# JuliaQuantumControl/QuOptimalControl.jl

Measured on AMD Instinct MI355X. Metric: GRAPE gradient-evals/sec, higher is better.
Workload: dtype f64; 1 GPU; C3: UnitaryGate 4x4, K=4, N=500 slices, ensemble E=1024 (one GPU, 1024 members/GPU), T=2.0; step = host->host grape_eval; parallelism=single GPU

## Files before the change

### quoptimalcontrol.jl_amd/csrc/grape_api.cpp

```cpp
#include "../../include/grape_hip.h"

#include <hip/hip_runtime.h>
#include <rccl/rccl.h>

#include <dlfcn.h>
#include <fcntl.h>
#include <time.h>
#include <unistd.h>

#include <algorithm>
#include <cmath>
#include <complex>
#include <cstdio>
#include <cstdlib>
#include <cstring>
#include <limits>
#include <atomic>
#include <condition_variable>
#include <mutex>
#include <thread>
#include <new>
#include <utility>
#include <string>
#include <vector>
// ... 21 lines not shown
    int any_blocks = 1;
    size_t scratch_bytes = 0;
    bool grid = false;
    int EU = 0;
    int S = 0, W = 0, LT = 0;
    bool pair = false;
    int CH = 0;
    int MPB = 1, NB = 0;
    int B = 1;
    double *d_block_out = nullptr;
    double *d_xg_scratch = nullptr;
    int ksplit = 1;
    size_t ws_elems = 0;
    int Ec = 0, EUc = 0;
    size_t ws_unit = 0;
    size_t ws_budget = 0;
    int ws_arrays = 1;
    bool ws_invalid = false;
    bool ws_keep_costates = false;
    int test_fail_replan = 0;
    int ws_B = 1;
    uint64_t bytes = 0;
    double2 *d_ops = nullptr;
    double *d_wts = nullptr;
    double *d_x = nullptr;
    double *d_fg = nullptr;
    double2 *d_props = nullptr, *d_states = nullptr, *d_costates = nullptr;
    double *d_zphi = nullptr;
    bool exact_w1 = false;
    double *d_member_out = nullptr;
    double *d_partial = nullptr;
    double *d_fom_member = nullptr, *d_fom_rows = nullptr;
    unsigned long long *d_stamps = nullptr;
    double *h_stage = nullptr;
    double *d_h_stage = nullptr;
    double *h_fg = nullptr;
    double *d_h_fg = nullptr;
    unsigned long long *h_flag = nullptr, *d_h_flag = nullptr;
    int mf_wait = 0;
    unsigned *d_done_counter = nullptr;
    bool peer_sum = false;
    bool peer_direct = false;
    bool peer_all = false;
    double *d_gather = nullptr;
    hipEvent_t ev_done = nullptr;
    unsigned *d_arrive = nullptr;
// ... 399 lines not shown
        if (w->th.joinable()) w->th.join();
        delete w;
        c->worker = nullptr;
    }
    for (grape_ctx *s : c->sub) free_all(s);
    c->sub.clear();
    if (c->is_group) {
        if (c->d_gather) { (void)hipSetDevice(c->device); (void)hipFree(c->d_gather); }
        if (c->d_arrive) { (void)hipSetDevice(c->device); (void)hipFree(c->d_arrive); }
        if (c->d_basis_phi) { (void)hipSetDevice(c->device); (void)hipFree(c->d_basis_phi); (void)hipFree(c->d_basis_x0); }
        if (c->d_bounds || c->d_slope) { (void)hipSetDevice(c->device); (void)hipFree(c->d_bounds); (void)hipFree(c->d_slope); }
        delete c;
        return;
    }
    (void)hipSetDevice(c->device);
    for (int j = 0; j < c->ipc_ranks; ++j)
        if (c->ipc_mbox[j] && c->ipc_mbox[j] != c->d_mbox) (void)hipIpcCloseMemHandle(c->ipc_mbox[j]);
    if (c->d_mbox) (void)hipFree(c->d_mbox);
    if (c->comm && g_rccl.handle) (void)g_rccl.CommDestroy(c->comm);
    for (hipEvent_t e : c->ev) (void)hipEventDestroy(e);
    if (c->ev_dev) (void)hipEventDestroy(c->ev_dev);
    if (c->ev_done) (void)hipEventDestroy(c->ev_done);
    if (c->stream) (void)hipStreamDestroy(c->stream);
    (void)hipFree(c->d_ops); (void)hipFree(c->d_wts); (void)hipFree(c->d_x); (void)hipFree(c->d_fg);
    (void)hipFree(c->d_props); (void)hipFree(c->d_states); (void)hipFree(c->d_costates); (void)hipFree(c->d_zphi);
    (void)hipFree(c->d_ctrl_scale);
    (void)hipFree(c->d_member_out); (void)hipFree(c->d_partial); (void)hipFree(c->d_stamps); (void)hipFree(c->d_block_out); (void)hipFree(c->d_xg_scratch);
    if (c->h_stage) (void)hipHostFree(c->h_stage);
    if (c->h_fg) (void)hipHostFree(c->h_fg);
    if (c->h_flag) (void)hipHostFree(c->h_flag);
    (void)hipFree(c->d_done_counter);
    (void)hipFree(c->d_scratch);
    (void)hipFree(c->d_vecs);
    (void)hipFree(c->d_sp_coef); (void)hipFree(c->d_sp_addr);
    (void)hipFree(c->d_any_sp_i); (void)hipFree(c->d_any_sp_c);
    (void)hipFree(c->d_tp_q); (void)hipFree(c->d_tp_r); (void)hipFree(c->d_tp_m); (void)hipFree(c->d_tp_z); (void)hipFree(c->d_tp_vec); (void)hipFree(c->d_tp_a);
    (void)hipFree(c->d_x_bar);
    (void)hipFree(c->d_pen_w);
    (void)hipFree(c->d_rc_R); (void)hipFree(c->d_rc_rho); (void)hipFree(c->d_rc_xs); (void)hipFree(c->d_rc_rows);
    (void)hipFree(c->d_obs_O); (void)hipFree(c->d_obs_y); (void)hipFree(c->d_obs_xf);
    (void)hipFree(c->d_vjp_O); (void)hipFree(c->d_vjp_ybar); (void)hipFree(c->d_vjp_xbar); (void)hipFree(c->d_vjp_part); (void)hipFree(c->d_vjp_g); (void)hipFree(c->d_vjp_out);
    (void)hipFree(c->d_traj_w); (void)hipFree(c->d_traj_x);
    (void)hipFree(c->d_jvp_O); (void)hipFree(c->d_jvp_xdot); (void)hipFree(c->d_jvp_xphys); (void)hipFree(c->d_jvp_ydot); (void)hipFree(c->d_jvp_xf);
    (void)hipFree(c->d_basis_phi); (void)hipFree(c->d_basis_x0);
    (void)hipFree(c->d_bounds); (void)hipFree(c->d_slope);
    (void)hipFree(c->d_fom_member); (void)hipFree(c->d_fom_rows);
    (void)hipFree(c->d_risk_rows); (void)hipFree(c->d_risk_p);
// ... 247 lines not shown
    if (e == hipSuccess && c->family == 0) e = alloc((void **)&c->d_block_out, sizeof(double) * c->NB * Q * Bn);
    if (e == hipSuccess && c->family == 0 && !xg_in_lds)
        e = alloc((void **)&c->d_xg_scratch,
                  sizeof(double) * Bn * c->NB * ((size_t)c->MPB * c->CH * ((size_t)S * K + 1) + c->MPB));
    if (e == hipSuccess && (cfg->flags & GRAPE_FLAG_PHASE_STAMPS)) {
        const size_t sb = sizeof(unsigned long long) * Bn * E * W * grape::kStampSlots;
        e = alloc((void **)&c->d_stamps, sb);
        if (e == hipSuccess) e = hipMemset(c->d_stamps, 0, sb);
    }
    const unsigned hflags = hipHostMallocMapped | hipHostMallocCoherent | hipHostMallocPortable;
    if (e == hipSuccess) e = hipHostMalloc((void **)&c->h_stage, sizeof(double) * Q * Bn, hflags);
    if (e == hipSuccess) e = hipHostGetDevicePointer((void **)&c->d_h_stage, c->h_stage, 0);
    if (e == hipSuccess) e = hipHostMalloc((void **)&c->h_fg, sizeof(double) * Q * Bn, hflags);
    if (e == hipSuccess) e = hipHostGetDevicePointer((void **)&c->d_h_fg, c->h_fg, 0);
    if (e == hipSuccess) e = hipHostMalloc((void **)&c->h_flag, 64 + sizeof(unsigned long long) * grape::kMaxMflags, hflags);
    if (e == hipSuccess) e = hipHostGetDevicePointer((void **)&c->d_h_flag, c->h_flag, 0);
    if (e == hipSuccess) { std::memset(c->h_flag, 0, 64 + sizeof(unsigned long long) * grape::kMaxMflags); e = alloc((void **)&c->d_done_counter, 64); }
    if (e == hipSuccess) e = hipMemset(c->d_done_counter, 0, 64);
    {
        const char *dp = std::getenv("GRAPE_DIRECT_PUBLISH");
        c->direct_publish = !(dp && dp[0] == '0');
        c->mf_publish = !env_off("GRAPE_MF_PUBLISH");
        c->pair_ah_env = !env_off("GRAPE_PAIR_AH");
    }
    {
        const char *xu = std::getenv("GRAPE_X_UPLOAD");
        int mode = 2;
        if (xu) mode = !std::strcmp(xu, "memcpy") ? 0 : (!std::strcmp(xu, "kernel") ? 1 : 2);
        int large_bar = 0;
        if (mode == 2 && e == hipSuccess &&
            (hipDeviceGetAttribute(&large_bar, hipDeviceAttributeIsLargeBar, dev) != hipSuccess || !large_bar))
            mode = 1;
        if (mode == 2 && e == hipSuccess) {
            void *p = nullptr;
            if (hipExtMallocWithFlags(&p, sizeof(double) * KN(c) * Bn, hipDeviceMallocFinegrained) == hipSuccess && p) {
                const int fd = open("/dev/zero", O_RDONLY);
                const bool ok = fd >= 0 && read(fd, p, 64) == 64;
                if (fd >= 0) close(fd);
                if (ok) {
                    c->d_x_bar = (double *)p;
                    c->bytes += sizeof(double) * KN(c) * Bn;
                } else {
                    (void)hipFree(p);
                    mode = 1;
                }
            } else {
// ... 1186 lines not shown
        if (c->tp_C) {
            const size_t bytes = sizeof(double2) * nn * (size_t)c->cfg.n_ensemble * c->B * (size_t)c->tp_C;
            const char *what = "the time chunks' products";
            if (int rc = grow(c, &c->d_tp_q, &c->tp_cap[0], bytes, who, what)) return rc;
            if (int rc = grow(c, &c->d_tp_r, &c->tp_cap[1], bytes, who, what)) return rc;
            if (int rc = grow(c, &c->d_tp_m, &c->tp_cap[2], bytes, who, what)) return rc;
        }
        const size_t need = per_block * (size_t)std::max(c->any_blocks, std::max(1, c->tp_C));
        if (int rc = grow(c, &c->d_scratch, &c->scratch_bytes, need, who, "the propagator blocks' scratch matrices")) return rc;
    }
    if (thin) {
        c->unitary = false;
        if (!c->d_vecs) {
            c->bytes += sizeof(double) * E * 4 * VS;
            HIP_TRY(c, hipMalloc((void **)&c->d_vecs, sizeof(double) * E * 4 * VS));
        }
        HIP_TRY(c, hipMemcpy(c->d_vecs, vecs.data(), sizeof(double) * E * 4 * VS, hipMemcpyHostToDevice));
        const size_t rec = sizeof(double2) * (size_t)c->Ec * ((size_t)c->cfg.n_slices + 1) * VS * ws_batch(c);
        if (int rc = grow(c, &c->d_states, &c->states_bytes, rec, who, "the forward states")) return rc;
    } else if (!herm || c->exact_w1) {
        if (int rc = grow(c, &c->d_states, &c->states_bytes, sizeof(double2) * c->ws_elems * ws_batch(c), who, "the forward states")) return rc;
    }
    HIP_TRY(c, hipMemcpy(c->d_ops, packed.data(), sizeof(double) * packed.size(), hipMemcpyHostToDevice));
    HIP_TRY(c, hipMemcpy(c->d_wts, wts, sizeof(double) * E, hipMemcpyHostToDevice));
    c->h_wts.assign(wts, wts + E);
    c->ops_set = true;
    c->evaluated = false;
    c->risk_evaluated = false;
    return GRAPE_OK;
}

static TileParams tile_params(const grape_ctx *c, const double *d_x, int n_x = 1)
{
    TileParams p{};
    p.n_x = n_x;
    p.ops = c->d_ops;
    p.x = d_x;
    p.props = c->d_props;
    p.states = c->d_states;
    p.costates = c->d_costates;
    p.member_out = c->d_member_out;
    p.K = c->cfg.n_controls;
    p.N = c->cfg.n_slices;
    p.E = c->EU;
    p.E_plan = c->EU;
    p.E_members = c->cfg.n_ensemble;
// ... 74 lines not shown
    if (pen_active(c)) {
        d.pen_x = d_x;
        d.pen_w = c->d_pen_w;
        d.pen_K = c->cfg.n_controls;
        d.pen_N = c->cfg.n_slices;
    }
    return d;
}

static grape::DoneSignal host_signal(grape_ctx *s, double *host_out)
{
    grape::DoneSignal d;
    d.counter = s->d_done_counter;
    d.flag = s->d_h_flag;
    d.seq = ++s->seq;
    d.host_out = host_out;
    return d;
}

static SweepParams sweep_params(const grape_ctx *c, const double *d_x, int n_x)
{
    SweepParams p{};
    p.ops = c->d_ops;
    p.x = d_x;
    p.wts = c->d_wts;
    p.MPB = c->MPB;
    p.BPX = c->NB;
    p.n_x = n_x;
    p.sk_magic = (uint32_t)((1ull << 32) / ((uint64_t)c->S * c->cfg.n_controls)) + 1u;
    p.K = c->cfg.n_controls;
    p.N = c->cfg.n_slices;
    p.E = c->cfg.n_ensemble;
    p.S = c->S;
    p.LT = c->LT;
    p.s_forced = c->cfg.expm_squarings;
    p.variant = c->cfg.variant;
    p.dt = c->cfg.duration / c->cfg.n_slices;
    return p;
}

static bool pair_antiherm(const grape_ctx *c)
{
    return c->family == 0 && c->pair && c->unitary && c->cfg.n == 4 && c->cfg.sys_type == GRAPE_UNITARY_GATE && !c->exact_w1 &&
           c->cfg.gradient != GRAPE_GRADIENT_EXACT && c->pair_ah_env;
}

// ... 269 lines not shown
        const size_t slot = (size_t)(c->ev_issued % kEventRing);
        e0 = c->ev[3 * slot];
        e1 = c->ev[3 * slot + 2];
        if (c->family == 1 || (c->family == 2 && c->any_blocks > 1)) emid = c->ev[3 * slot + 1];
        c->ev_has_mid[slot] = emid ? 1 : 0;
        c->ev_issued += 1;
        HIP_TRY(c, hipEventRecord(e0, stream));
    }
    const bool exact = c->cfg.gradient == GRAPE_GRADIENT_EXACT;
    if (exact) p.member_out = nullptr;
    const bool direct = c->family == 0 && c->NB == 1 && n_x == 1 && !exact && c->direct_publish && !done.probe_out &&
                        !done.stage_base && !pen_active(c) && !rc_on && !risk;
    const bool fold = !done.stage_base && tile_folds_reduce(c, n_x);
    if (direct) {
        p.direct_dst = done.flag && done.host_out ? done.host_out : d_fg;
        p.direct_flag = done.flag;
        p.direct_seq = done.seq;
    }
    const size_t nn = (size_t)c->cfg.n * c->cfg.n, Kc = (size_t)c->cfg.n_controls, Qrow = KN(c) + 1;
    auto launch_members = [&](int lo, int cnt) -> int {
        if (c->family == 0) {
            SweepParams q = p;
            q.ops = p.ops + (size_t)lo * (Kc + 3) * nn;
            q.wts = p.wts + lo;
            if (p.member_out) q.member_out = p.member_out + (size_t)lo * Qrow;
            q.block_out = p.block_out + (size_t)(lo / c->MPB) * Qrow;
            if (p.zphi) q.zphi = p.zphi + 2 * (size_t)lo;
            q.E = cnt;
            q.BPX = (cnt + c->MPB - 1) / c->MPB;
            const int mode = c->unitary ? 2 : (c->d_costates ? 1 : 0), sand = c->cfg.sys_type != GRAPE_UNITARY_GATE;
            HIP_TRY(c, launch_small_family(c, sand, (mode == 2 && pair_antiherm(c)) ? 3 : mode, q, stream));
            if (rc_on) {
                SweepParams r = q;
                r.rc_only = 1;
                r.rc_terms = c->rc_terms;
                r.rc_m = c->m;
                r.rc_unitary = c->unitary ? 1 : 0;
                r.rc_CH = c->CH;
                r.rc_Etot = c->cfg.n_ensemble;
                r.rc_R = c->d_rc_R + (size_t)lo * c->cfg.n * c->m;
                r.rc_rho = c->d_rc_rho;
                r.rc_xs = c->d_rc_xs;
                r.rc_rows = c->d_rc_rows;
                if (c->rc_mode == GRAPE_TRAJ_EXACT) {
                    r.rc_exact = 1;
                    r.traj_w = c->d_traj_w;
// ... 2126 lines not shown
```

### quoptimalcontrol.jl_amd/csrc/grape_kernels.hpp

```cpp
#pragma once
#include <hip/hip_runtime.h>
#include <stddef.h>
#include <stdint.h>
#include <type_traits>

namespace grape {

void log_kernel(const char *expr);
#define GRAPE_LAUNCH(KERNEL, ...)                        \
    do {                                                 \
        ::grape::log_kernel(#KERNEL);                    \
        hipLaunchKernelGGL(KERNEL, __VA_ARGS__);         \
    } while (0)
#define GRAPE_LAUNCH_AS(NAME, KERNEL, ...)               \
    do {                                                 \
        ::grape::log_kernel(NAME);                       \
        hipLaunchKernelGGL(KERNEL, __VA_ARGS__);         \
    } while (0)


constexpr double kTheta8 = 0.08;

struct BasisOp {
    int32_t project = 0;
// ... 8 lines not shown
};
struct DoneSignal {
    unsigned *counter = nullptr;
    unsigned long long *flag = nullptr;
    unsigned long long seq = 0;
    double *host_out = nullptr;
    const double *stage_base = nullptr;
    int n_total = 0;
    const double *probe_dir = nullptr;
    const double *probe_sc = nullptr;
    double *probe_out = nullptr;
    unsigned long long *mflags = nullptr;
    const double *pen_x = nullptr;
    const double *pen_w = nullptr;
    int pen_K = 0, pen_N = 0;
    const BasisOp *basis = nullptr;
    double risk_beta = 0.0;
    double *risk_p = nullptr;
    double *risk_F = nullptr;
};
constexpr int kMaxMflags = 1000;
int reduce_rows_mflags(int Q, int n_x);

constexpr int kStampSlots = 8;

struct SweepParams {
    const double2 *ops;
    const double *x;
    double2 *props;
    double2 *states;
    double2 *costates;
    double *member_out;
    const double *wts;
    double *block_out;
    unsigned long long *stamps;
    double *xg_scratch;
    int32_t K, N, E;
    int32_t S;
    int32_t LT;
    int32_t MPB;
    int32_t BPX;
    int32_t n_x;
    uint32_t sk_magic;
    int32_t s_forced;
    int32_t variant;
    int32_t plast_lds;
    double dt;
// ... 44 lines not shown
    double *vjp_part;
    double *vjp_G;
    int32_t obs_staged;
    int32_t vjp_staged;
    int32_t jvp_only;
    int32_t jvp_n;
    int32_t jvp_m;
    int32_t jvp_per_member;
    int32_t jvp_CH;
    int32_t jvp_Etot;
    int32_t jvp_E0;
    const double2 *jvp_O;
    const double *jvp_xdot;
    double2 *jvp_ydot;
    double2 *jvp_xf;
    int32_t traj_exact;
    double2 *traj_w;
    const double *traj_x;
    int32_t rc_exact;
    int32_t rc_unweighted;
    int32_t jvp_ndir;
    int32_t jvp_multi;
    int64_t jvp_dir_xdot, jvp_dir_ydot, jvp_dir_xf, jvp_dir_w;
};
constexpr int kJvpMultiMaxThreads = 256;
constexpr int jvp_multi_block(int n, int m)
{
    return n == 2 ? 8 : n == 3 ? 4 : n == 4 ? (m <= 2 ? 3 : 2) : 0;
}
constexpr bool jvp_multi_default(int n, int m)
{
    return jvp_multi_block(n, m) > 0;
}
constexpr int traj_max_threads(int n)
{
    return n == 2 ? 1024 : n == 3 ? 512 : 256;
}
constexpr size_t traj_static_lds(int n, int m, bool vjp)
{
    return (size_t)(traj_max_threads(n) / 64) * (size_t)(n * n + (vjp ? n * m : 0)) * 16;
}
template <typename F>
hipError_t dispatch_nm(int n, int m, F &&f)
{
#define GRAPE_NM_CASE(N, M) \
    case N * 8 + M: return f(std::integral_constant<int, N>{}, std::integral_constant<int, M>{})
    switch (n * 8 + m) {
// ... 225 lines not shown
```

### quoptimalcontrol.jl_amd/csrc/sweep_pair.hip

```cpp
#include "cmatp.hpp"
#include "grape_kernels.hpp"

#ifndef GRAPE_ABL
#define GRAPE_ABL 0
#endif
#ifndef GRAPE_PD
#define GRAPE_PD 2
#endif
#ifndef GRAPE_PLAYOUT
#define GRAPE_PLAYOUT 0
#endif
#ifndef GRAPE_PD_EARLY
#define GRAPE_PD_EARLY 2
#endif
#ifndef GRAPE_PD_EARLY_AT
#define GRAPE_PD_EARLY_AT 0
#endif
#ifndef GRAPE_MBAR
#define GRAPE_MBAR 2
#endif

namespace grape {

enum { PMODE_GENERAL = 0, PMODE_GENERAL_KEEPL = 1, PMODE_UNITARY = 2, PMODE_UNITARY_AH = 3 };
constexpr int kAhImage = 5;
constexpr int kParityPad = 8;

template <int N>
GRAPE_DEV int gelem(int q, int r, int jl)
{
    constexpr int NC = N / 2;
    const int i = (((r / NC) ^ q) * NC) + (r % NC);
    const int j = q * NC + jl;
    return i + j * N;
}

template <int N>
GRAPE_DEV void pstore_ws(double2 *__restrict__ base, size_t stride, const PMat<N> &m, int q)
{
#pragma unroll
    for (int jl = 0; jl < N / 2; ++jl)
#pragma unroll
        for (int r = 0; r < N; ++r)
            base[(size_t)gelem<N>(q, r, jl) * stride] = make_double2(m.re[r + jl * N], m.im[r + jl * N]);
}

template <int N>
GRAPE_DEV void pstore_ws_split(double2 *__restrict__ sbase, const unsigned (&voff)[2], size_t stride, const PMat<N> &m)
{
// ... 191 lines not shown
    for (int c = 0; c < K; c += 2) {
        if (c + 1 < K) {
#pragma unroll
            for (int e = 0; e < kAhImage; ++e)
                b1[e] = s_img[(c + 1) * kAhImage + e];
        }
        const double re = dot(b0);
        if (p == 0)
            out[c] = gs * re;
        if (c + 1 < K) {
            if (c + 2 < K) {
#pragma unroll
                for (int e = 0; e < kAhImage; ++e)
                    b0[e] = s_img[(c + 2) * kAhImage + e];
            }
            const double r1 = dot(b1);
            if (p == 0)
                out[c + 1] = gs * r1;
        }
    }
}

constexpr int kVecSlices = 16;
template <int N, int SAND, int MODE, int MAXT, bool XGLDS, bool DUMPW = false, bool VEC = false>
__global__ __launch_bounds__(MAXT) void sweep_pair_kernel(const double2 *__restrict__ ops_all,
                                                          const double *__restrict__ x_all,
                                                          const double *__restrict__ wts_all,
                                                          const SweepParams p)
{
    constexpr int NN = N * N, NC = N / 2, NE = N * NC;
    constexpr int MAXW = MAXT / 64;
    constexpr bool AH = (MODE == PMODE_UNITARY_AH);
    constexpr bool UNI = (MODE == PMODE_UNITARY) || AH;
    constexpr bool KEEPL = (MODE == PMODE_GENERAL_KEEPL);
    static_assert(!AH || (N == 4 && !SAND && !DUMPW && !VEC), "the anti-Hermitian sweep serves UnitaryGate at n = 4, first-order gradient");
    constexpr bool PDASM = (GRAPE_PD == 2) && UNI && N == 4 && !DUMPW && XGLDS;
    extern __shared__ double2 s_dyn[];
    double2(*s_tot)[MAXW][NN] = reinterpret_cast<double2(*)[MAXW][NN]>(s_dyn);

    const int LT = p.LT, W = LT >> 6, CH = LT >> 1;
    const int mb = __builtin_amdgcn_readfirstlane(threadIdx.x / LT);
    const int L = threadIdx.x - mb * LT;
    const int lane = L & 63, wave = L >> 6;
    const int par = L & 1;
    const int ch = L >> 1;
    const int cw = lane >> 1;
    const int wbase_tot = mb * W;
    const int xi = blockIdx.x / p.BPX;
    const int bi = blockIdx.x - xi * p.BPX;
    int kl = bi * p.MPB + mb;
    const bool valid = kl < p.E;
    if (!valid)
        kl = p.E - 1;
    const int k = xi * p.E + kl;
    const int K = p.K, Nsl = p.N, S = p.S;
    const size_t stride = (size_t)CH;
    const int NM = 2 * K + 4;

    unsigned *s_cnt = reinterpret_cast<unsigned *>(s_dyn + 2 * MAXW * NN);
    double2 *s_ops_all = s_dyn + 2 * MAXW * NN + 4;
    const int PS = NM * NE + kParityPad;
    double2 *s_ops = s_ops_all + (size_t)mb * 2 * PS;
    const int SK = S * K;
    const size_t nrm_d2 = ((size_t)p.MPB * (K + 1) + 1) / 2;
    double *s_xg_all = XGLDS ? reinterpret_cast<double *>(s_ops_all + (size_t)p.MPB * 2 * PS + nrm_d2)
                             : p.xg_scratch + (size_t)blockIdx.x * ((size_t)p.MPB * CH * (SK + 1) + p.MPB);
    double *s_xg = s_xg_all + (size_t)mb * CH * (SK + 1);
    double *s_F = s_xg_all + (size_t)p.MPB * CH * (SK + 1);
    double2 *s_plast = reinterpret_cast<double2 *>(s_F + ((p.MPB + 1) & ~1));
    double *s_nrm = reinterpret_cast<double *>(s_ops_all + (size_t)p.MPB * 2 * PS) + (size_t)mb * (K + 1);
    const unsigned magic = p.sk_magic;
    auto chunk_of = [&](int q) { return SK == 1 ? q : (int)__umulhi((unsigned)q, magic); };
    if (threadIdx.x < 16)
        s_cnt[threadIdx.x] = 0u;
    if (p.tune & 7) {
        const int sel = p.tune & 7;
        const bool hi = sel == 1 ? (mb & 1) : sel == 2 ? (mb & 2) : sel == 3 ? (blockIdx.x & 1) : sel == 4 ? ((threadIdx.x >> 6) & 1) : false;
        if (hi)
            __builtin_amdgcn_s_setprio(2);
    }
    {
        const double *__restrict__ xsrc = x_all + (size_t)xi * K * Nsl;
        const int KNs = K * Nsl;
        for (int q0 = 0; q0 < KNs; q0 += 8 * LT) {
            double v[8];
#pragma unroll
            for (int u = 0; u < 8; ++u) {
                const int q = q0 + u * LT + L;
                v[u] = q < KNs ? xsrc[q] : 0.0;
            }
#pragma unroll
            for (int u = 0; u < 8; ++u) {
                const int q = q0 + u * LT + L;
                if (q < KNs)
                    s_xg[q + chunk_of(q)] = v[u];
            }
        }
        const double2 *__restrict__ ops = ops_all + (size_t)kl * (K + 3) * NN;
        for (int idx = L; idx < 2 * NM * NE; idx += LT) {
            const int q = idx / (NM * NE), rem = idx - q * NM * NE;
            const int mat = rem / NE, e = rem - mat * NE;
            if (mat == 2 * K + 3 || (AH && mat > K && mat <= 2 * K))
                continue;
// ... 34 lines not shown
        double sr = 0.0, si = 0.0;
        for (int kk = 0; kk < N; ++kk) {
            const double2 a = gXi[i + kk * N], b = gXt[j + kk * N];
            sr = fma(a.x, b.x, sr); sr = fma(a.y, b.y, sr);
            si = fma(a.y, b.x, si); si = fma(-a.x, b.y, si);
        }
        s_ops[(size_t)q * PS + (size_t)(2 * K + 3) * NE + e] = make_double2(sr, si);
    }
    __syncthreads();
    if (L <= K) {
        double best = 0.0;
        for (int q = 0; q < 2; ++q)
            for (int jl = 0; jl < NC; ++jl) {
                double cs = 0.0;
                for (int r = 0; r < N; ++r) {
                    const double2 v = s_ops[(size_t)q * PS + (size_t)L * NE + r + jl * N];
                    cs += fabs(v.x) + fabs(v.y);
                }
                best = fmax(best, cs);
            }
        s_nrm[L] = best;
    }
    __syncthreads();
    const double2 *sA = s_ops + (size_t)par * PS;
    const double2 *sB = sA + NE;
    const double2 *sBT = sA + (size_t)(1 + K) * NE;
    const double2 *sXi = sA + (size_t)(1 + 2 * K) * NE;
    const double2 *sXt = sXi + NE;
    const double2 *sXi_o = s_ops + (size_t)(1 - par) * PS + (size_t)(1 + 2 * K) * NE;
    const double2 *sXt_o = sXi_o + NE;
    const double2 *sXX = sXt + NE, *sXX_o = sXt_o + NE;
    double *xg = s_xg + ch * (SK + 1);
    const size_t wbase = (size_t)k * S * NN * stride + ch;
    const size_t pstep = GRAPE_PLAYOUT ? (size_t)p.E * p.n_x * NN * stride : (size_t)NN * stride;
    double2 *__restrict__ Pw = p.props + (GRAPE_PLAYOUT ? (size_t)k * NN * stride + ch : wbase);
    double2 *__restrict__ Xw = p.states + wbase;
    double *__restrict__ out = p.member_out + (size_t)k * ((size_t)K * Nsl + 1);
    const int t0 = ch * S;
    const unsigned p_rowb = (unsigned)CH * 16u;
    const unsigned p_voff[2] = {(unsigned)(par * NC + par * NC * N) * p_rowb + (unsigned)ch * 16u,
                                (unsigned)((1 - par) * NC + par * NC * N) * p_rowb + (unsigned)ch * 16u};
    double2 *__restrict__ const p_Pk = p.props + (size_t)k * (GRAPE_PLAYOUT ? 1 : S) * NN * stride;
    unsigned long long *__restrict__ st =
        p.stamps ? p.stamps + ((size_t)k * W + wave) * kStampSlots : nullptr;
    if (st && lane == 0)
        st[5] = __builtin_amdgcn_s_memrealtime();
    pstamp(st, 0);

    PMat<N> Q, Q2;
    auto build = [&](int j, PMat<N> &G) -> double {
        double nb = s_nrm[0];
        double2 b0[NE], b1[NE];
#pragma unroll
        for (int e = 0; e < NE; ++e)
            b0[e] = sB[e];
        if (p.variant != 0)
            pload_lds(G, sA);
        for (int c = 0; c < K; c += 2) {
            const int c1 = min(c + 1, K - 1), c2 = min(c + 2, K - 1);
            const double x0 = xg[j * K + c];
            const double x1 = (c + 1 < K) ? xg[j * K + c1] : 0.0;
            nb = fma(fabs(x0), s_nrm[1 + c], nb);
            nb = fma(fabs(x1), s_nrm[1 + c1], nb);
#pragma unroll
            for (int e = 0; e < NE; ++e)
                b1[e] = sB[c1 * NE + e];
            if (c == 0 && p.variant == 0) {
#pragma unroll
                for (int e = 0; e < NE; ++e) {
// ... 681 lines not shown
            for (int m = 0; m < nmem; ++m) {
                const double v = (q < KN) ? s_xg_all[m * mstride + off] : s_F[m];
                acc = fma(v, wb[m], acc);
            }
            bout[q] = acc;
            if (p.direct_dst)
                p.direct_dst[q] = acc;
        }
    }
    if (p.direct_flag) {
        __threadfence_system();
        __syncthreads();
        if (threadIdx.x == 0)
            __hip_atomic_store(p.direct_flag, p.direct_seq, __ATOMIC_RELEASE, __HIP_MEMORY_SCOPE_SYSTEM);
    }
    pstamp(st, 4);
    if (st && lane == 0) {
        st[6] = __builtin_amdgcn_s_memrealtime();
        st[7] = ((unsigned long long)__builtin_amdgcn_s_getreg(20 | (31 << 11)) << 32) |
                (unsigned)__builtin_amdgcn_s_getreg(4 | (31 << 11));
    }
}

template <int N>
struct PairTraits;
template <> struct PairTraits<2> { static constexpr int MAXT = 1024; };
template <> struct PairTraits<4> { static constexpr int MAXT = 512; };

int sweep_pair_max_waves(int n)
{
    switch (n) {
    case 2: return PairTraits<2>::MAXT / 64;
    case 4: return PairTraits<4>::MAXT / 64;
    default: return 0;
    }
}

size_t sweep_pair_lds_bytes(int n, int MPB, int LT, int S, int K, bool xg_in_lds, bool plast)
{
    const int maxt = n == 2 ? PairTraits<2>::MAXT : PairTraits<4>::MAXT;
    size_t b = sizeof(double2) * (2 * (size_t)(maxt / 64) * n * n + 4);
    b += sizeof(double2) * ((size_t)MPB * 2 * ((2 * K + 4) * (n * (n / 2)) + kParityPad) + ((size_t)MPB * (K + 1) + 1) / 2);
    if (xg_in_lds)
        b += sizeof(double) * ((size_t)MPB * (LT / 2) * ((size_t)S * K + 1) + ((MPB + 1) & ~1));
    if (plast)
        b += sizeof(double2) * (size_t)MPB * LT * (n * (n / 2));
    return b;
}

template <int N, int SAND, int MODE, bool XGLDS>
static hipError_t plaunch_one(const SweepParams &p0, hipStream_t stream)
{
    constexpr int MAXT = PairTraits<N>::MAXT;
    SweepParams p = p0;
    const dim3 grid(p.BPX * p.n_x), block(p.LT * p.MPB);
    size_t lds = sweep_pair_lds_bytes(N, p.MPB, p.LT, p.S, p.K, XGLDS);
    if (lds > 160 * 1024)
        return hipErrorInvalidConfiguration;
    p.plast_lds = 0;
    {
        static const int tune_env = [] { const char *e = getenv("GRAPE_PAIR_TUNE"); return e ? atoi(e) : 0; }();
        p.tune = tune_env;
    }
    if ((MODE == PMODE_UNITARY || MODE == PMODE_UNITARY_AH) && XGLDS && p.S > 1) {
        const size_t with = sweep_pair_lds_bytes(N, p.MPB, p.LT, p.S, p.K, true, true);
        if (with <= 160 * 1024) {
            p.plast_lds = 1;
            lds = with;
        }
    }
    if constexpr (MODE == PMODE_UNITARY && SAND == 0) {
        if (p.dump_w1) {
            auto kern_w = sweep_pair_kernel<N, SAND, MODE, MAXT, XGLDS, true>;
            if (lds > 64 * 1024) {
                hipError_t e = ensure_dynamic_lds((const void *)kern_w, lds);
                if (e != hipSuccess)
                    return e;
            }
            GRAPE_LAUNCH_AS("sweep_pair_kernel", kern_w, grid, block, lds, stream, p.ops, p.x, p.wts, p);
            return hipGetLastError();
        }
    }
    if (p.dump_w1)
        return hipErrorInvalidConfiguration;
    if constexpr (N == 4 && SAND == 0 && MODE == PMODE_GENERAL && XGLDS) {
        if (p.vec && p.S <= kVecSlices) {
            auto kern_v = sweep_pair_kernel<N, SAND, MODE, MAXT, XGLDS, false, true>;
            if (lds > 64 * 1024) {
                hipError_t e = ensure_dynamic_lds((const void *)kern_v, lds);
                if (e != hipSuccess)
                    return e;
            }
            GRAPE_LAUNCH_AS("sweep_pair_vec_kernel", kern_v, grid, block, lds, stream, p.ops, p.x, p.wts, p);
            return hipGetLastError();
        }
    }
    auto kern = sweep_pair_kernel<N, SAND, MODE, MAXT, XGLDS>;
    if (lds > 64 * 1024) {
        hipError_t e = ensure_dynamic_lds((const void *)kern, lds);
        if (e != hipSuccess)
            return e;
    }
    GRAPE_LAUNCH_AS("sweep_pair_kernel", kern, grid, block, lds, stream, p.ops, p.x, p.wts, p);
    return hipGetLastError();
}

template <int N, int SAND>
static hipError_t plaunch_ns(int mode, const SweepParams &p, hipStream_t stream)
{
    constexpr int MAXT = PairTraits<N>::MAXT;
    if (p.MPB < 1 || p.LT * p.MPB > MAXT || (p.LT & 63) || (long long)p.S * (p.LT / 2) < p.N)
        return hipErrorInvalidConfiguration;
    const bool lds = p.xg_scratch == nullptr;
    switch (mode) {
    case PMODE_GENERAL:
        return lds ? plaunch_one<N, SAND, PMODE_GENERAL, true>(p, stream) : plaunch_one<N, SAND, PMODE_GENERAL, false>(p, stream);
    case PMODE_GENERAL_KEEPL:
        return lds ? plaunch_one<N, SAND, PMODE_GENERAL_KEEPL, true>(p, stream)
                   : plaunch_one<N, SAND, PMODE_GENERAL_KEEPL, false>(p, stream);
    case PMODE_UNITARY:
        return lds ? plaunch_one<N, SAND, PMODE_UNITARY, true>(p, stream) : plaunch_one<N, SAND, PMODE_UNITARY, false>(p, stream);
    case PMODE_UNITARY_AH:
        if constexpr (N == 4 && SAND == 0)
            return lds ? plaunch_one<N, SAND, PMODE_UNITARY_AH, true>(p, stream)
                       : plaunch_one<N, SAND, PMODE_UNITARY_AH, false>(p, stream);
        return hipErrorInvalidConfiguration;
    default:
        return hipErrorInvalidValue;
    }
}

hipError_t launch_sweep_pair(int n, int sandwich, int mode, const SweepParams &p, hipStream_t stream)
{
    if (p.fom_only)
        return launch_fom_small(n, sandwich, mode, true, p, stream);
    if (p.rc_only)
        return run_running_cost(n, p, stream);
    if (p.obs_only)
        return run_observe(n, sandwich, p, stream);
    if (p.vjp_only)
        return run_trajectory_vjp(n, p, stream);
    if (p.jvp_only)
        return run_trajectory_jvp(n, p, stream);
    switch (n * 2 + (sandwich ? 1 : 0)) {
    case 4: return plaunch_ns<2, 0>(mode, p, stream);
    case 5: return plaunch_ns<2, 1>(mode, p, stream);
    case 8: return plaunch_ns<4, 0>(mode, p, stream);
    case 9: return plaunch_ns<4, 1>(mode, p, stream);
    default: return hipErrorInvalidValue;
    }
}

}
```

### quoptimalcontrol.jl_amd/engine.py

```python
import ctypes as C
import os
import subprocess

import numpy as np

_HERE = os.path.dirname(os.path.abspath(__file__))
_LIB = None

SYS_TYPE_CODES = {"UnitaryGate": 0, "StateTransfer": 1, "CoherenceTransfer": 2}
FLAG_KEEP_COSTATES = 1
FLAG_TIME_KERNELS = 2
FLAG_PHASE_STAMPS = 4
FLAG_FORCE_GENERAL = 8
FLAG_MEMBER_RESULTS = 16
FLAG_FORCE_COLLECTIVE = 32
FLAG_TIME_SAMPLED = 64
FLAG_GROUP_PEER_SUM = 128
MAX_DEVICES = 8
MAX_JVP_DIRECTIONS = 8
ABI_VERSION = 8

STATUS = {0: "GRAPE_OK", -1: "GRAPE_ERR_INVALID_ARG", -2: "GRAPE_ERR_UNSUPPORTED",
          -3: "GRAPE_ERR_NO_DEVICE", -4: "GRAPE_ERR_HIP", -5: "GRAPE_ERR_NOT_READY",
          -6: "GRAPE_ERR_ALLOC", -7: "GRAPE_ERR_TIMEOUT", -8: "GRAPE_ERR_COMM"}
# ... 732 lines not shown
        self._check(self._lib.grape_eval_batch_device(self._h, int(n_x), C.c_void_p(d_x_ptr), C.c_void_p(d_fg_ptr),
                                                      C.c_void_p(stream)))

    def member_results(self):
        foms = np.empty(self.E)
        grads = np.empty((self.E, self.N, self.K))
        self._check(self._lib.grape_get_member_results(self._h, _p(foms), _p(grads)))
        return foms, np.ascontiguousarray(np.swapaxes(grads, 1, 2))

    def trajectory(self, member, costates=False, states=True):
        n, N, m = self.n, self.N, self.m
        P = np.empty((N, n, n), np.complex128)
        X = np.empty((N + 1, m, n), np.complex128) if states else None
        Lc = np.empty((N + 1, m, n), np.complex128) if costates else None
        self._check(self._lib.grape_get_trajectory(self._h, int(member), _p(P), _p(X), _p(Lc)))
        sw = lambda a: None if a is None else np.ascontiguousarray(np.swapaxes(a, -1, -2))
        return (sw(P), sw(X), sw(Lc)) if costates else (sw(P), sw(X))

    def phase_stamps(self):
        cnt = C.c_int64()
        self._check(self._lib.grape_get_phase_stamps(self._h, None, 0, C.byref(cnt)))
        out = np.empty(cnt.value, dtype=np.uint64)
        self._check(self._lib.grape_get_phase_stamps(self._h, _p(out), cnt.value, C.byref(cnt)))
        return out.reshape(-1, 8)

    def group_timing(self, reset=False):
        out = np.zeros(6)
        self._check(self._lib.grape_get_group_timing(self._h, _p(out), int(reset)))
        return dict(zip(("evaluations", "stage_x_us", "issue_skew_us", "sum_issue_us", "wait_us", "total_us"), out.tolist()))

    def kernel_samples(self, capacity=65536):
        cnt = C.c_int64()
        self._check(self._lib.grape_get_kernel_samples(self._h, None, None, 0, C.byref(cnt)))
        n = min(int(cnt.value), int(capacity))
        tot, first = np.empty(n), np.empty(n)
        if n:
            self._check(self._lib.grape_get_kernel_samples(self._h, _p(tot), _p(first), n, C.byref(cnt)))
        return tot, first

    def kernel_names(self):
        need = self._lib.grape_get_kernel_names(self._h, None, 0)
        if need < 0:
            self._check(need)
        buf = C.create_string_buffer(max(int(need), 1))
        self._check(min(self._lib.grape_get_kernel_names(self._h, buf, len(buf)), 0))
        return [k for k in buf.value.decode().split(";") if k]

# ... 6 lines not shown
```

Baseline: 12370 gradient-evals/s.

## Precompute per-member pair operator image once at set_ops and copy it into LDS

A new kernel builds each ensemble member's LDS operator image (rearranged control/drift blocks, anti-Hermitian weights, column norms) once, when operators are uploaded. The sweep kernel then does a straight batched copy of that image and the controls into shared memory instead of rebuilding it on every gradient evaluation. This removes per-eval prologue arithmetic and scattered global reads, at the cost of extra device memory and a second kernel variant. It also adds two entry timestamp slots to the phase stamps.

```diff
diff --git a/quoptimalcontrol.jl_amd/csrc/grape_api.cpp b/quoptimalcontrol.jl_amd/csrc/grape_api.cpp
--- a/quoptimalcontrol.jl_amd/csrc/grape_api.cpp
+++ b/quoptimalcontrol.jl_amd/csrc/grape_api.cpp
@@ -67,6 +67,8 @@
     int ws_B = 1;
     uint64_t bytes = 0;
     double2 *d_ops = nullptr;
+    double2 *d_pair_img = nullptr;
+    bool pair_image_env = true;
     double *d_wts = nullptr;
     double *d_x = nullptr;
     double *d_fg = nullptr;
@@ -512,7 +514,7 @@
     if (c->ev_dev) (void)hipEventDestroy(c->ev_dev);
     if (c->ev_done) (void)hipEventDestroy(c->ev_done);
     if (c->stream) (void)hipStreamDestroy(c->stream);
-    (void)hipFree(c->d_ops); (void)hipFree(c->d_wts); (void)hipFree(c->d_x); (void)hipFree(c->d_fg);
+    (void)hipFree(c->d_ops); (void)hipFree(c->d_pair_img); (void)hipFree(c->d_wts); (void)hipFree(c->d_x); (void)hipFree(c->d_fg);
     (void)hipFree(c->d_props); (void)hipFree(c->d_states); (void)hipFree(c->d_costates); (void)hipFree(c->d_zphi);
     (void)hipFree(c->d_ctrl_scale);
     (void)hipFree(c->d_member_out); (void)hipFree(c->d_partial); (void)hipFree(c->d_stamps); (void)hipFree(c->d_block_out); (void)hipFree(c->d_xg_scratch);
@@ -806,6 +808,7 @@
         c->direct_publish = !(dp && dp[0] == '0');
         c->mf_publish = !env_off("GRAPE_MF_PUBLISH");
         c->pair_ah_env = !env_off("GRAPE_PAIR_AH");
+        c->pair_image_env = !env_off("GRAPE_PAIR_IMAGE");
     }
     {
         const char *xu = std::getenv("GRAPE_X_UPLOAD");
@@ -2038,6 +2041,21 @@
         if (int rc = grow(c, &c->d_states, &c->states_bytes, sizeof(double2) * c->ws_elems * ws_batch(c), who, "the forward states")) return rc;
     }
     HIP_TRY(c, hipMemcpy(c->d_ops, packed.data(), sizeof(double) * packed.size(), hipMemcpyHostToDevice));
+    if (c->family == 0 && c->pair && c->pair_image_env) {
+        const size_t ib = sizeof(double2) * (size_t)grape::pair_image_d2(c->cfg.n, c->cfg.n_controls) * E;
+        if (!c->d_pair_img) {
+            c->bytes += ib;
+            HIP_TRY(c, hipMalloc((void **)&c->d_pair_img, ib));
+        }
+        SweepParams ip{};
+        ip.ops = c->d_ops;
+        ip.pair_img = c->d_pair_img;
+        ip.img_only = 1;
+        ip.K = c->cfg.n_controls;
+        ip.E = c->cfg.n_ensemble;
+        HIP_TRY(c, grape::launch_sweep_pair(c->cfg.n, 0, 0, ip, nullptr));
+        HIP_TRY(c, hipStreamSynchronize(nullptr));
+    }
     HIP_TRY(c, hipMemcpy(c->d_wts, wts, sizeof(double) * E, hipMemcpyHostToDevice));
     c->h_wts.assign(wts, wts + E);
     c->ops_set = true;
@@ -2158,6 +2176,7 @@
 {
     SweepParams p{};
     p.ops = c->d_ops;
+    p.pair_img = c->d_pair_img;
     p.x = d_x;
     p.wts = c->d_wts;
     p.MPB = c->MPB;
@@ -2473,6 +2492,7 @@
         if (c->family == 0) {
             SweepParams q = p;
             q.ops = p.ops + (size_t)lo * (Kc + 3) * nn;
+            if (p.pair_img) q.pair_img = p.pair_img + (size_t)lo * grape::pair_image_d2(c->cfg.n, (int)Kc);
             q.wts = p.wts + lo;
             if (p.member_out) q.member_out = p.member_out + (size_t)lo * Qrow;
             q.block_out = p.block_out + (size_t)(lo / c->MPB) * Qrow;
diff --git a/quoptimalcontrol.jl_amd/csrc/grape_kernels.hpp b/quoptimalcontrol.jl_amd/csrc/grape_kernels.hpp
--- a/quoptimalcontrol.jl_amd/csrc/grape_kernels.hpp
+++ b/quoptimalcontrol.jl_amd/csrc/grape_kernels.hpp
@@ -54,7 +54,7 @@
 constexpr int kMaxMflags = 1000;
 int reduce_rows_mflags(int Q, int n_x);
 
-constexpr int kStampSlots = 8;
+constexpr int kStampSlots = 10;
 
 struct SweepParams {
     const double2 *ops;
@@ -145,7 +145,13 @@
     int32_t jvp_ndir;
     int32_t jvp_multi;
     int64_t jvp_dir_xdot, jvp_dir_ydot, jvp_dir_xf, jvp_dir_w;
-};
+    double2 *pair_img;
+    int32_t img_only;
+};
+constexpr int kParityPad = 8;
+constexpr int pair_image_ps(int n, int K) { return (2 * K + 4) * (n * (n / 2)) + kParityPad; }
+constexpr int pair_image_nrm_at(int n, int K) { return (n == 4 ? 4 : 2) * pair_image_ps(n, K); }
+constexpr int pair_image_d2(int n, int K) { return pair_image_nrm_at(n, K) + (K + 2) / 2; }
 constexpr int kJvpMultiMaxThreads = 256;
 constexpr int jvp_multi_block(int n, int m)
 {
diff --git a/quoptimalcontrol.jl_amd/csrc/sweep_pair.hip b/quoptimalcontrol.jl_amd/csrc/sweep_pair.hip
--- a/quoptimalcontrol.jl_amd/csrc/sweep_pair.hip
+++ b/quoptimalcontrol.jl_amd/csrc/sweep_pair.hip
@@ -24,7 +24,6 @@
 
 enum { PMODE_GENERAL = 0, PMODE_GENERAL_KEEPL = 1, PMODE_UNITARY = 2, PMODE_UNITARY_AH = 3 };
 constexpr int kAhImage = 5;
-constexpr int kParityPad = 8;
 
 template <int N>
 GRAPE_DEV int gelem(int q, int r, int jl)
@@ -262,11 +261,12 @@
 }
 
 constexpr int kVecSlices = 16;
-template <int N, int SAND, int MODE, int MAXT, bool XGLDS, bool DUMPW = false, bool VEC = false>
-__global__ __launch_bounds__(MAXT) void sweep_pair_kernel(const double2 *__restrict__ ops_all,
-                                                          const double *__restrict__ x_all,
-                                                          const double *__restrict__ wts_all,
-                                                          const SweepParams p)
+
+constexpr int kPairXBatch = 16, kPairImgBatch = 4;
+
+template <int N, int SAND, int MODE, int MAXT, bool XGLDS, bool DUMPW, bool VEC, bool IMG>
+GRAPE_DEV void sweep_pair_body(const double2 *__restrict__ ops_all, const double *__restrict__ x_all,
+                               const double *__restrict__ wts_all, const SweepParams &p)
 {
     constexpr int NN = N * N, NC = N / 2, NE = N * NC;
     constexpr int MAXW = MAXT / 64;
@@ -277,6 +277,11 @@
     constexpr bool PDASM = (GRAPE_PD == 2) && UNI && N == 4 && !DUMPW && XGLDS;
     extern __shared__ double2 s_dyn[];
     double2(*s_tot)[MAXW][NN] = reinterpret_cast<double2(*)[MAXW][NN]>(s_dyn);
+    unsigned long long t_in_real = 0, t_in_cyc = 0;
+    if (p.stamps) {
+        t_in_real = __builtin_amdgcn_s_memrealtime();
+        t_in_cyc = __builtin_readcyclecounter();
+    }
 
     const int LT = p.LT, W = LT >> 6, CH = LT >> 1;
     const int mb = __builtin_amdgcn_readfirstlane(threadIdx.x / LT);
@@ -319,6 +324,34 @@
         if (hi)
             __builtin_amdgcn_s_setprio(2);
     }
+    if constexpr (IMG) {
+        const double *__restrict__ xsrc = x_all + (size_t)xi * K * Nsl;
+        const int KNs = K * Nsl, REC = 2 * PS;
+        const double2 *__restrict__ rec0 = p.pair_img + (size_t)kl * pair_image_d2(N, K);
+        const double2 *__restrict__ rec = rec0 + (AH ? REC : 0);
+        const double *__restrict__ rnrm = reinterpret_cast<const double *>(rec0 + pair_image_nrm_at(N, K));
+        double v[kPairXBatch];
+        d2v im[kPairImgBatch];
+        const int sk1 = SK == 1 ? -1 : 0;
+#pragma unroll
+        for (int u = 0; u < kPairImgBatch; ++u)
+            im[u] = reinterpret_cast<const d2v *>(rec)[min(u * LT + L, REC - 1)];
+        const double nr = rnrm[min(L, K)];
+#pragma unroll
+        for (int u = 0; u < kPairXBatch; ++u)
+            v[u] = xsrc[min(u * LT + L, KNs - 1)];
+        __builtin_amdgcn_sched_barrier(0);
+#pragma unroll
+        for (int u = 0; u < kPairImgBatch; ++u)
+            reinterpret_cast<d2v *>(s_ops)[min(u * LT + L, REC - 1)] = im[u];
+        s_nrm[min(L, K)] = nr;
+#pragma unroll
+        for (int u = 0; u < kPairXBatch; ++u) {
+            const int q = min(u * LT + L, KNs - 1);
+            s_xg[q + (int)__umulhi((unsigned)q, magic) + (q & sk1)] = v[u];
+        }
+        __syncthreads();
+    } else {
     {
         const double *__restrict__ xsrc = x_all + (size_t)xi * K * Nsl;
         const int KNs = K * Nsl;
@@ -399,6 +432,7 @@
         s_nrm[L] = best;
     }
     __syncthreads();
+    }
     const double2 *sA = s_ops + (size_t)par * PS;
     const double2 *sB = sA + NE;
     const double2 *sBT = sA + (size_t)(1 + K) * NE;
@@ -419,9 +453,12 @@
                                 (unsigned)((1 - par) * NC + par * NC * N) * p_rowb + (unsigned)ch * 16u};
     double2 *__restrict__ const p_Pk = p.props + (size_t)k * (GRAPE_PLAYOUT ? 1 : S) * NN * stride;
     unsigned long long *__restrict__ st =
-        p.stamps ? p.stamps + ((size_t)k * W + wave) * kStampSlots : nullptr;
-    if (st && lane == 0)
+        p.stamps ? p.stamps + ((size_t)k * W + __builtin_amdgcn_readfirstlane(wave)) * kStampSlots : nullptr;
+    if (st && lane == 0) {
+        st[8] = t_in_real;
+        st[9] = t_in_cyc;
         st[5] = __builtin_amdgcn_s_memrealtime();
+    }
     pstamp(st, 0);
 
     PMat<N> Q, Q2;
@@ -1149,6 +1186,114 @@
     }
 }
 
+template <int N, int SAND, int MODE, int MAXT, bool XGLDS, bool DUMPW = false, bool VEC = false>
+__global__ __launch_bounds__(MAXT) void sweep_pair_kernel(const double2 *__restrict__ ops_all,
+                                                          const double *__restrict__ x_all,
+                                                          const double *__restrict__ wts_all,
+                                                          const SweepParams p)
+{
+    sweep_pair_body<N, SAND, MODE, MAXT, XGLDS, DUMPW, VEC, XGLDS>(ops_all, x_all, wts_all, p);
+}
+
+template <int N, int SAND, int MODE, int MAXT, bool XGLDS, bool DUMPW = false, bool VEC = false>
+__global__ __launch_bounds__(MAXT) void sweep_pair_build_kernel(const double2 *__restrict__ ops_all,
+                                                                const double *__restrict__ x_all,
+                                                                const double *__restrict__ wts_all,
+                                                                const SweepParams p)
+{
+    sweep_pair_body<N, SAND, MODE, MAXT, XGLDS, DUMPW, VEC, false>(ops_all, x_all, wts_all, p);
+}
+
+template <int N>
+__global__ __launch_bounds__(64) void pair_image_kernel(const double2 *__restrict__ ops_all, double2 *__restrict__ img_all,
+                                                        int K, int E)
+{
+    constexpr int NN = N * N, NC = N / 2, NE = N * NC;
+    constexpr bool AH = (N == 4);
+    const int kl = blockIdx.x, L = threadIdx.x, LT = blockDim.x;
+    if (kl >= E)
+        return;
+    const int NM = 2 * K + 4, PS = pair_image_ps(N, K), REC = 2 * PS;
+    const double2 *__restrict__ ops = ops_all + (size_t)kl * (K + 3) * NN;
+    double2 *__restrict__ rec = img_all + (size_t)kl * pair_image_d2(N, K);
+    auto ah_weight = [&](int q, int c, int sl) {
+        const int P0 = q * NC, Q0 = (1 - q) * NC;
+        int jj, ii;
+        double wt = 1.0;
+        if (sl < 2)       { jj = ii = P0 + sl; }
+        else if (sl < 4)  { jj = P0 + 1; ii = P0; wt = 2.0; }
+        else if (sl < 6)  { jj = P0; ii = Q0; }
+        else if (sl < 8)  { jj = P0 + 1; ii = Q0 + 1; }
+        else              { jj = P0 + 1; ii = Q0; wt = 2.0; }
+        const double2 b1 = ops[(size_t)(1 + c) * NN + jj + ii * N], b2 = ops[(size_t)(1 + c) * NN + ii + jj * N];
+        const double bsr = 0.5 * (b1.x - b2.x), bsi = 0.5 * (b1.y + b2.y);
+        const double v = sl < 2 ? -bsi : ((sl & 1) ? -wt * bsi : wt * bsr);
+        return v;
+    };
+    for (int idx = L; idx < REC; idx += LT) {
+        const int q = idx / PS, rem = idx - q * PS;
+        const int mat = rem / NE, e = rem - mat * NE;
+        double2 val = make_double2(0.0, 0.0), val_ah = val;
+        if (mat == 2 * K + 3) {
+            const double2 *__restrict__ gXi = ops + (size_t)(1 + K) * NN, *__restrict__ gXt = gXi + NN;
+            const int r = e % N, jl = e / N;
+            const int i = (((r / NC) ^ q) * NC) + (r % NC), j = q * NC + jl;
+            double sr = 0.0, si = 0.0;
+            for (int kk = 0; kk < N; ++kk) {
+                const double2 a = gXi[i + kk * N], b = gXt[j + kk * N];
+                sr = fma(a.x, b.x, sr); sr = fma(a.y, b.y, sr);
+                si = fma(a.y, b.x, si); si = fma(-a.x, b.y, si);
+            }
+            val = val_ah = make_double2(sr, si);
+        } else if (mat < NM) {
+            const int r = e % N, jl = e / N;
+            const int i = (((r / NC) ^ q) * NC) + (r % NC), j = q * NC + jl;
+            int src;
+            if (mat <= K)            src = mat * NN + i + j * N;
+            else if (mat <= 2 * K)   src = (mat - K) * NN + j + i * N;
+            else                     src = (mat - K) * NN + i + j * N;
+            val = val_ah = ops[src];
+            if (AH && mat > K && mat <= 2 * K) {
+                const int d0 = 2 * (rem - (1 + K) * NE);
+                val_ah = make_double2(0.0, 0.0);
+                if (d0 < K * 2 * kAhImage) {
+                    const int c = d0 / (2 * kAhImage), sl = d0 - c * (2 * kAhImage);
+                    val_ah = make_double2(ah_weight(q, c, sl), ah_weight(q, c, sl + 1));
+                }
+            }
+        }
+        rec[idx] = val;
+        if (AH)
+            rec[REC + idx] = val_ah;
+    }
+    if (L <= K) {
+        double best = 0.0;
+        for (int q = 0; q < 2; ++q)
+            for (int jl = 0; jl < NC; ++jl) {
+                double cs = 0.0;
+                for (int r = 0; r < N; ++r) {
+                    const double2 v = ops[(size_t)L * NN + gelem<N>(q, r, jl)];
+                    cs += fabs(v.x) + fabs(v.y);
+                }
+                best = fmax(best, cs);
+            }
+        reinterpret_cast<double *>(rec + pair_image_nrm_at(N, K))[L] = best;
+    }
+}
+
+static hipError_t run_pair_image(int n, const SweepParams &p, hipStream_t stream)
+{
+    if (!p.pair_img || p.E < 1)
+        return hipErrorInvalidValue;
+    if (n == 2)
+        GRAPE_LAUNCH_AS("pair_image_kernel", pair_image_kernel<2>, dim3(p.E), dim3(64), 0, stream, p.ops, p.pair_img, p.K, p.E);
+    else if (n == 4)
+        GRAPE_LAUNCH_AS("pair_image_kernel", pair_image_kernel<4>, dim3(p.E), dim3(64), 0, stream, p.ops, p.pair_img, p.K, p.E);
+    else
+        return hipErrorInvalidValue;
+    return hipGetLastError();
+}
+
 template <int N>
 struct PairTraits;
 template <> struct PairTraits<2> { static constexpr int MAXT = 1024; };
@@ -1173,6 +1318,15 @@
     if (plast)
         b += sizeof(double2) * (size_t)MPB * LT * (n * (n / 2));
     return b;
+}
+
+template <int N, int SAND, int MODE, int MAXT, bool XGLDS, bool DUMPW, bool VEC>
+static auto pair_build_kernel()
+{
+    if constexpr (XGLDS)
+        return sweep_pair_build_kernel<N, SAND, MODE, MAXT, XGLDS, DUMPW, VEC>;
+    else
+        return sweep_pair_kernel<N, SAND, MODE, MAXT, XGLDS, DUMPW, VEC>;
 }
 
 template <int N, int SAND, int MODE, bool XGLDS>
@@ -1196,40 +1350,31 @@
             lds = with;
         }
     }
+    const bool copy = XGLDS && p.pair_img && (long long)p.K * p.N <= (long long)kPairXBatch * p.LT &&
+                      2 * pair_image_ps(N, p.K) <= kPairImgBatch * p.LT;
+    auto go = [&](auto kern_copy, auto kern_build, const char *name) -> hipError_t {
+        auto kern = copy ? kern_copy : kern_build;
+        if (lds > 64 * 1024) {
+            hipError_t e = ensure_dynamic_lds((const void *)kern, lds);
+            if (e != hipSuccess)
+                return e;
+        }
+        GRAPE_LAUNCH_AS(name, kern, grid, block, lds, stream, p.ops, p.x, p.wts, p);
+        return hipGetLastError();
+    };
     if constexpr (MODE == PMODE_UNITARY && SAND == 0) {
         if (p.dump_w1) {
-            auto kern_w = sweep_pair_kernel<N, SAND, MODE, MAXT, XGLDS, true>;
-            if (lds > 64 * 1024) {
-                hipError_t e = ensure_dynamic_lds((const void *)kern_w, lds);
-                if (e != hipSuccess)
-                    return e;
-            }
-            GRAPE_LAUNCH_AS("sweep_pair_kernel", kern_w, grid, block, lds, stream, p.ops, p.x, p.wts, p);
-            return hipGetLastError();
+            return go(sweep_pair_kernel<N, SAND, MODE, MAXT, XGLDS, true>, pair_build_kernel<N, SAND, MODE, MAXT, XGLDS, true, false>(), "sweep_pair_kernel");
         }
     }
     if (p.dump_w1)
         return hipErrorInvalidConfiguration;
     if constexpr (N == 4 && SAND == 0 && MODE == PMODE_GENERAL && XGLDS) {
         if (p.vec && p.S <= kVecSlices) {
-            auto kern_v = sweep_pair_kernel<N, SAND, MODE, MAXT, XGLDS, false, true>;
-            if (lds > 64 * 1024) {
-                hipError_t e = ensure_dynamic_lds((const void *)kern_v, lds);
-                if (e != hipSuccess)
-                    return e;
-            }
-            GRAPE_LAUNCH_AS("sweep_pair_vec_kernel", kern_v, grid, block, lds, stream, p.ops, p.x, p.wts, p);
-            return hipGetLastError();
-        }
-    }
-    auto kern = sweep_pair_kernel<N, SAND, MODE, MAXT, XGLDS>;
-    if (lds > 64 * 1024) {
-        hipError_t e = ensure_dynamic_lds((const void *)kern, lds);
-        if (e != hipSuccess)
-            return e;
-    }
-    GRAPE_LAUNCH_AS("sweep_pair_kernel", kern, grid, block, lds, stream, p.ops, p.x, p.wts, p);
-    return hipGetLastError();
+            return go(sweep_pair_kernel<N, SAND, MODE, MAXT, XGLDS, false, true>, pair_build_kernel<N, SAND, MODE, MAXT, XGLDS, false, true>(), "sweep_pair_vec_kernel");
+        }
+    }
+    return go(sweep_pair_kernel<N, SAND, MODE, MAXT, XGLDS>, pair_build_kernel<N, SAND, MODE, MAXT, XGLDS, false, false>(), "sweep_pair_kernel");
 }
 
 template <int N, int SAND>
@@ -1259,6 +1404,8 @@
 
 hipError_t launch_sweep_pair(int n, int sandwich, int mode, const SweepParams &p, hipStream_t stream)
 {
+    if (p.img_only)
+        return run_pair_image(n, p, stream);
     if (p.fom_only)
         return launch_fom_small(n, sandwich, mode, true, p, stream);
     if (p.rc_only)
diff --git a/quoptimalcontrol.jl_amd/engine.py b/quoptimalcontrol.jl_amd/engine.py
--- a/quoptimalcontrol.jl_amd/engine.py
+++ b/quoptimalcontrol.jl_amd/engine.py
@@ -778,7 +778,7 @@
         self._check(self._lib.grape_get_phase_stamps(self._h, None, 0, C.byref(cnt)))
         out = np.empty(cnt.value, dtype=np.uint64)
         self._check(self._lib.grape_get_phase_stamps(self._h, _p(out), cnt.value, C.byref(cnt)))
-        return out.reshape(-1, 8)
+        return out.reshape(-1, 10)
 
     def group_timing(self, reset=False):
         out = np.zeros(6)
```

After: 12880 gradient-evals/s, median of 6. 1.04x the previous value.
